# voidstrike/FPSG

Measured on AMD Instinct MI355X. Metric: episodes/sec (+ Chamfer-kernel HBM GB/s in roofline.hbm), 2048-pt clouds, 224x224 images; episode = fwd + Chamfer + bwd, step = E episodes + all-reduce + Adam, higher is better.
Workload: dtype f32

## Files before the change

fpsg_amd/csrc/conv_first.hip:

```cpp
#include "fpsg_common.h"

namespace fpsg {
namespace {

constexpr int kFirstThreads = 256;

struct FoldArgs {
  const float* y;
  const float* chan;
  const float* coef;
  const float* pre_bias;
};

template <int PX, bool FOLD>
__global__ __launch_bounds__(kFirstThreads) void conv_first_dw_kernel(const float* __restrict__ x,
                                                                      const float* __restrict__ dy, FoldArgs fa, int H, int W,
                                                                      int segs_per_row, int n_segs,
                                                                      float* __restrict__ part ) {
  constexpr int LD = PX + 4;
  constexpr int VPR = PX / 4;
  constexpr int NV = 64 * VPR / kFirstThreads;
  constexpr int PE = 9 * (PX + 2);
  constexpr int NP = (PE + kFirstThreads - 1) / kFirstThreads;
  static_assert(64 * VPR % kFirstThreads == 0, "tile vectors divide over the threads");
  __shared__ float dyt[64 * LD];
  __shared__ float xt[9 * LD];
  const int tid = threadIdx.x, lane = tid & 63, wave = tid >> 6;
  const int kk = lane >> 4, col = lane & 15;
  int boff[2];
  bool bval[2];
#pragma unroll
  for (int nt = 0; nt < 2; ++nt) {
    const int tap = 16 * nt + col;
    bval[nt] = tap < 27;
    const int t = bval[nt] ? tap : 0;
    boff[nt] = (t / 3) * LD + (t % 3);
  }
  int vch[NV], vq4[NV], pcr[NP], pj[NP];
#pragma unroll
  for (int it = 0; it < NV; ++it) {
    const int v = it * kFirstThreads + tid;
    vch[it] = v / VPR;
    vq4[it] = (v - vch[it] * VPR) * 4;
  }
#pragma unroll
  for (int it = 0; it < NP; ++it) {
    const int e = it * kFirstThreads + tid;
    pcr[it] = e < PE ? e / (PX + 2) : -1;
    pj[it] = e - (e / (PX + 2)) * (PX + 2);
  }
  v4f rv[NV];
  v4f ry[FOLD ? NV : 1];
  float rp[NP];
  float fsc[FOLD ? NV : 1], fsh[FOLD ? NV : 1], fk1[FOLD ? NV : 1], fk2[FOLD ? NV : 1], fk3[FOLD ? NV : 1], fb[FOLD ? NV : 1];
  if constexpr (FOLD) {
#pragma unroll
    for (int it = 0; it < NV; ++it) {
      const int c = vch[it];
      fsc[it] = fa.chan[c]; fsh[it] = fa.chan[64 + c];
      fk1[it] = fa.coef[c]; fk2[it] = fa.coef[64 + c]; fk3[it] = fa.coef[128 + c];
      fb[it] = fa.pre_bias ? fa.pre_bias[c] : 0.0f;
    }
  }
  auto fetch = [&](int seg) {
    const int row = seg / segs_per_row;
    const int w0 = (seg - row * segs_per_row) * PX;
    const int n = row / H;
    const int h = row - n * H;
#pragma unroll
    for (int it = 0; it < NV; ++it) {
      rv[it] = (v4f){0.0f, 0.0f, 0.0f, 0.0f};
      if constexpr (FOLD) ry[it] = rv[it];
      if (w0 + vq4[it] < W) {
        const size_t o = (((size_t)n * 64 + vch[it]) * H + h) * W + w0 + vq4[it];
        rv[it] = *reinterpret_cast<const v4f*>(dy + o);
        if constexpr (FOLD) ry[it] = *reinterpret_cast<const v4f*>(fa.y + o);
      } else if constexpr (FOLD) {
        ry[it] = (v4f){-3.0e38f, -3.0e38f, -3.0e38f, -3.0e38f};
      }
    }
#pragma unroll
    for (int it = 0; it < NP; ++it) {
      const int c = pcr[it] / 3, r = pcr[it] - 3 * c;
      const int hh = h + r - 1, ww = w0 + pj[it] - 1;
      rp[it] = 0.0f;
      if (pcr[it] >= 0 && hh >= 0 && hh < H && ww >= 0 && ww < W) rp[it] = x[(((size_t)n * 3 + c) * H + hh) * W + ww];
    }
  };
  v4f acc[2] = {{0.0f, 0.0f, 0.0f, 0.0f}, {0.0f, 0.0f, 0.0f, 0.0f}};
  int seg = blockIdx.x;
  if (seg < n_segs) fetch(seg);
  for (; seg < n_segs; seg += gridDim.x) {
    __syncthreads();
#pragma unroll
    for (int it = 0; it < NV; ++it) {
      v4f v = rv[it];
      if constexpr (FOLD) {
#pragma unroll
        for (int u = 0; u < 4; ++u) {
          const float xv = ry[it][u] + fb[it];
          const float dz = rv[it][u] * (fma_rn(xv, fsc[it], fsh[it]) > 0.0f ? 1.0f : 0.0f);
          const float dx = fma_rn(fk1[it], dz, fma_rn(fk2[it], xv, fk3[it]));
          v[u] = ry[it][u] == -3.0e38f ? 0.0f : dx;
        }
      }
      *reinterpret_cast<v4f*>(dyt + vch[it] * LD + vq4[it]) = v;
    }
#pragma unroll
    for (int it = 0; it < NP; ++it)
      if (pcr[it] >= 0) xt[pcr[it] * LD + pj[it]] = rp[it];
    __syncthreads();
    if (seg + (int)gridDim.x < n_segs) fetch(seg + gridDim.x);
    const float* ap = dyt + (16 * wave + col) * LD + kk;
    const float* bp0 = xt + boff[0] + kk;
    const float* bp1 = xt + boff[1] + kk;
#pragma unroll
    for (int s = 0; s < PX / 4; ++s) {
      const float a = ap[4 * s];
      const float b0 = bval[0] ? bp0[4 * s] : 0.0f;
      const float b1 = bval[1] ? bp1[4 * s] : 0.0f;
      acc[0] = __builtin_amdgcn_mfma_f32_16x16x4f32(a, b0, acc[0], 0, 0, 0);
      acc[1] = __builtin_amdgcn_mfma_f32_16x16x4f32(a, b1, acc[1], 0, 0, 0);
    }
  }
  float* pp = part + (size_t)blockIdx.x * 64 * 32;
#pragma unroll
  for (int nt = 0; nt < 2; ++nt)
#pragma unroll
    for (int r = 0; r < 4; ++r) pp[(16 * wave + 4 * kk + r) * 32 + 16 * nt + col] = acc[nt][r];
}

__global__ __launch_bounds__(1024) void conv_first_dw_reduce_kernel(const float* __restrict__ part, int n_part,
                                                                    float* __restrict__ dw ) {
  __shared__ double acc[32][32];
  const int k = blockIdx.x, tap = threadIdx.x & 31, g = threadIdx.x >> 5;
  double a = 0.0;
#pragma unroll 8
  for (int p = g; p < n_part; p += 32) a += (double)part[((size_t)p * 64 + k) * 32 + tap];
  acc[g][tap] = a;
  __syncthreads();
  if (g == 0 && tap < 27) {
    double t = acc[0][tap];
#pragma unroll
    for (int q = 1; q < 32; ++q) t += acc[q][tap];
    dw[k * 27 + tap] = (float)t;
  }
}


__device__ __forceinline__ void first_load_weights(const float* __restrict__ wt, const float* __restrict__ bias, int k,
                                                   float (&w)[27], float& b) {
#pragma unroll
  for (int i = 0; i < 27; ++i) w[i] = wt[k * 27 + i];
  b = bias ? bias[k] : 0.0f;
}

__device__ __forceinline__ void first_wait_weights(const float (&w)[27], float b) {
  asm volatile("" ::"s"(w[0]), "s"(w[15]), "s"(w[23]), "s"(w[25]), "s"(w[26]), "s"(b));
  __builtin_amdgcn_sched_barrier(0);
}

__device__ __forceinline__ void first_channel(const float (&d)[3][3][6], const float (&w)[27], float (&o)[4]) {
#pragma unroll
  for (int p = 0; p < 4; ++p) o[p] = 0.0f;
#pragma unroll
  for (int c = 0; c < 3; ++c)
#pragma unroll
    for (int a = 0; a < 3; ++a)
#pragma unroll
      for (int b = 0; b < 3; ++b) {
        const float wv = w[(c * 3 + a) * 3 + b];
#pragma unroll
        for (int p = 0; p < 4; ++p) o[p] = fma_rn(wv, d[c][a][b + p], o[p]);
      }
}

__device__ __forceinline__ void first_lane_sums(const float (&o)[4], float bk, bool live, float& s0, float& s1) {
  s0 = 0.0f;
  s1 = 0.0f;
#pragma unroll
  for (int p = 0; p < 4; ++p) {
    const float v = o[p] + bk;
    s0 += v;
    s1 = fma_rn(v, v, s1);
  }
  if (!live) s0 = s1 = 0.0f;
}

template <bool STATS, bool NT = false>
__global__ __launch_bounds__(kFirstThreads) void conv_first_fwd_kernel(const float* __restrict__ x,
                                                                       const float* __restrict__ wt , int H,
                                                                       int W, long Q, float* __restrict__ y,
                                                                       const float* __restrict__ bias,
                                                                       float* __restrict__ parts) {
  __shared__ float red[kFirstThreads / 64][64][2];
  const int tid = threadIdx.x, lane = tid & 63, wave = tid >> 6;
  const long q_raw = (long)blockIdx.x * kFirstThreads + tid;
  const bool live = q_raw < Q;
  const long q = live ? q_raw : Q - 1;
  const int W4 = W >> 2;
  const int w4 = (int)(q % W4);
  const long t = q / W4;
  const int h = (int)(t % H);
  const long n = t / H;
  const bool has_left = w4 > 0, has_right = w4 < W4 - 1;
  const bool left_lane = has_left && lane > 0, right_lane = has_right && lane < 63;
  v4f mid[3][3];
  float el[3][3], er[3][3];
  const float* rp[3][3];
  bool rin[3];
#pragma unroll
  for (int a = 0; a < 3; ++a) {
    const int r = h + a - 1;
    rin[a] = r >= 0 && r < H;
    const int rc = rin[a] ? r : h;
#pragma unroll
    for (int c = 0; c < 3; ++c) {
      rp[c][a] = x + (((size_t)n * 3 + c) * H + rc) * W + 4 * w4;
      mid[c][a] = *reinterpret_cast<const v4f*>(rp[c][a]);
      el[c][a] = er[c][a] = 0.0f;
    }
  }
  if (has_left && !left_lane) {
#pragma unroll
    for (int a = 0; a < 3; ++a)
#pragma unroll
      for (int c = 0; c < 3; ++c) el[c][a] = rp[c][a][-1];
  }
  if (has_right && !right_lane) {
#pragma unroll
    for (int a = 0; a < 3; ++a)
#pragma unroll
      for (int c = 0; c < 3; ++c) er[c][a] = rp[c][a][4];
  }
  float d[3][3][6];
#pragma unroll
  for (int c = 0; c < 3; ++c) {
#pragma unroll
    for (int a = 0; a < 3; ++a) {
      v4f m = mid[c][a];
      if (!rin[a]) m = (v4f){0.0f, 0.0f, 0.0f, 0.0f};
      float lft = __shfl_up(m[3], 1, 64), rgt = __shfl_down(m[0], 1, 64);
      if (!left_lane) lft = (has_left && rin[a]) ? el[c][a] : 0.0f;
      if (!right_lane) rgt = (has_right && rin[a]) ? er[c][a] : 0.0f;
      d[c][a][0] = lft; d[c][a][1] = m[0]; d[c][a][2] = m[1]; d[c][a][3] = m[2]; d[c][a][4] = m[3]; d[c][a][5] = rgt;
    }
  }
  const size_t plane = (size_t)H * W;
  float* yp = y + ((size_t)n * 64 * H + h) * W + 4 * w4;
  float wa[27], wb[27], ba = 0.0f, bb = 0.0f;
  first_load_weights(wt, STATS ? bias : nullptr, 0, wa, ba);
  for (int k = 0; k < 64; k += 2) {
    first_wait_weights(wa, ba);
    first_load_weights(wt, STATS ? bias : nullptr, k + 1, wb, bb);
    __builtin_amdgcn_sched_barrier(0);
    float oa[4], ob[4];
    first_channel(d, wa, oa);
    if (live) st_stream<NT>(reinterpret_cast<v4f*>(yp + (size_t)k * plane), (v4f){oa[0], oa[1], oa[2], oa[3]});
    float a0 = 0.0f, a1 = 0.0f, b0 = 0.0f, b1 = 0.0f;
    if (STATS) first_lane_sums(oa, ba, live, a0, a1);
    first_wait_weights(wb, bb);
    first_load_weights(wt, STATS ? bias : nullptr, k + 2 < 64 ? k + 2 : 63, wa, ba);
    __builtin_amdgcn_sched_barrier(0);
    first_channel(d, wb, ob);
    if (live) st_stream<NT>(reinterpret_cast<v4f*>(yp + (size_t)(k + 1) * plane), (v4f){ob[0], ob[1], ob[2], ob[3]});
    if (STATS) {
      first_lane_sums(ob, bb, live, b0, b1);
      wave_sum4_to_last(a0, a1, b0, b1);
      if (lane == 63) {
        *reinterpret_cast<v2f*>(&red[wave][k][0]) = (v2f){a0, a1};
        *reinterpret_cast<v2f*>(&red[wave][k + 1][0]) = (v2f){b0, b1};
      }
    }
  }
  if (STATS) {
    __syncthreads();
    if (tid < 64) {
      float t0 = red[0][tid][0], t1 = red[0][tid][1];
#pragma unroll
      for (int w2 = 1; w2 < kFirstThreads / 64; ++w2) { t0 += red[w2][tid][0]; t1 += red[w2][tid][1]; }
      float* out = parts + ((size_t)tid * gridDim.x + blockIdx.x) * 2;
      out[0] = t0;
      out[1] = t1;
    }
  }
}

}
}

extern "C" size_t fpsg_conv_first_dw_workspace_floats(int N, int H, int W) {
  if (N <= 0 || H <= 0 || W <= 0) return 0;
  return (size_t)2048 * 64 * 32;
}

static int conv_first_dw_launch(const char* fn, const float* x, const float* dy, fpsg::FoldArgs fa, int N, int C, int K,
                                int H, int W, float* dw, float* ws, fpsg_stream_t stream) {
  using namespace fpsg;
  const bool fold = fa.y != nullptr;
  FPSG_REQUIRE(C == 3 && K == 64, FPSG_E_SHAPE, "%s: the 3 -> 64 channel layer only (got %d -> %d)", fn, C, K);
  FPSG_REQUIRE(N > 0 && H > 0 && W > 0 && W % 4 == 0, FPSG_E_SHAPE,
               "%s: N, H positive and W a positive multiple of 4 (got %d,%d,%d)", fn, N, H, W);
  FPSG_REQUIRE_PTR(x); FPSG_REQUIRE_PTR(dy); FPSG_REQUIRE_PTR(dw); FPSG_REQUIRE_PTR(ws);
  FPSG_REQUIRE((reinterpret_cast<uintptr_t>(dy) & 15) == 0 && (reinterpret_cast<uintptr_t>(fa.y) & 15) == 0, FPSG_E_ALIGN,
               "%s: dy / y / ga must be 16-byte aligned", fn);
  hipStream_t s = static_cast<hipStream_t>(stream);
  const int px = W % 112 == 0 ? 112 : 64;
  const int segs_per_row = (W + px - 1) / px;
  const long n_segs_l = (long)N * H * segs_per_row;
  FPSG_REQUIRE(n_segs_l < (1L << 31), FPSG_E_LIMIT, "fpsg_conv_first_dw: %ld row segments beyond the 32-bit walk", n_segs_l);
  const int n_segs = (int)n_segs_l;
  const int resident = px == 112 ? 1024 : 2048;
  const int blocks = n_segs < resident ? n_segs : resident;
  if (px == 112 && fold)
    hipLaunchKernelGGL((conv_first_dw_kernel<112, true>), dim3(blocks), dim3(kFirstThreads), 0, s, x, dy, fa, H, W, segs_per_row, n_segs, ws);
  else if (px == 112)
    hipLaunchKernelGGL((conv_first_dw_kernel<112, false>), dim3(blocks), dim3(kFirstThreads), 0, s, x, dy, fa, H, W, segs_per_row, n_segs, ws);
  else if (fold)
    hipLaunchKernelGGL((conv_first_dw_kernel<64, true>), dim3(blocks), dim3(kFirstThreads), 0, s, x, dy, fa, H, W, segs_per_row, n_segs, ws);
  else
    hipLaunchKernelGGL((conv_first_dw_kernel<64, false>), dim3(blocks), dim3(kFirstThreads), 0, s, x, dy, fa, H, W, segs_per_row, n_segs, ws);
  int rc = launch_status(fn);
  if (rc) return rc;
  hipLaunchKernelGGL(conv_first_dw_reduce_kernel, dim3(64), dim3(1024), 0, s, ws, blocks, dw);
  return launch_status(fn);
}

extern "C" int fpsg_conv_first_dw(const float* x, const float* dy, int N, int C, int K, int H, int W, float* dw,
                                  float* ws, fpsg_stream_t stream) {
  return conv_first_dw_launch("fpsg_conv_first_dw", x, dy, fpsg::FoldArgs{nullptr, nullptr, nullptr, nullptr}, N, C, K, H, W,
                              dw, ws, stream);
}

extern "C" int fpsg_conv_first_dw_fold(const float* x, const float* y, const float* ga, const float* chan,
                                       const float* coef, const float* pre_bias, int N, int C, int K, int H, int W,
                                       float* dw, float* ws, fpsg_stream_t stream) {
  using namespace fpsg;
  FPSG_REQUIRE_PTR(y); FPSG_REQUIRE_PTR(chan); FPSG_REQUIRE_PTR(coef);
  FPSG_REQUIRE(!misaligned4(pre_bias), FPSG_E_ALIGN, "fpsg_conv_first_dw_fold: pre_bias not 4-byte aligned");
  return conv_first_dw_launch("fpsg_conv_first_dw_fold", x, ga, FoldArgs{y, chan, coef, pre_bias}, N, C, K, H, W, dw, ws,
                              stream);
}

extern "C" int fpsg_conv_first_parts(int N, int H, int W) {
  if (N <= 0 || H <= 0 || W <= 0 || W % 4) return 0;
  const long Q = (long)N * H * (W / 4);
  return (int)((Q + fpsg::kFirstThreads - 1) / fpsg::kFirstThreads);
}

extern "C" int fpsg_conv_first_fwd(const float* x, const float* w, int N, int C, int K, int H, int W, float* y,
                                   const float* bias, float* parts, fpsg_stream_t stream) {
  using namespace fpsg;
  FPSG_REQUIRE(C == 3 && K == 64, FPSG_E_SHAPE, "fpsg_conv_first_fwd: the 3 -> 64 channel layer only (got %d -> %d)", C, K);
  FPSG_REQUIRE(N > 0 && H > 0 && W > 0 && W % 4 == 0, FPSG_E_SHAPE,
               "fpsg_conv_first_fwd: N, H positive and W a positive multiple of 4 (got %d,%d,%d)", N, H, W);
  FPSG_REQUIRE_PTR(x); FPSG_REQUIRE_PTR(w); FPSG_REQUIRE_PTR(y);
  FPSG_REQUIRE(((reinterpret_cast<uintptr_t>(x) | reinterpret_cast<uintptr_t>(y)) & 15) == 0, FPSG_E_ALIGN,
               "fpsg_conv_first_fwd: x and y must be 16-byte aligned");
  FPSG_REQUIRE(!misaligned4(bias) && !misaligned4(parts) && !misaligned4(w), FPSG_E_ALIGN,
               "fpsg_conv_first_fwd: w / bias / parts not 4-byte aligned");
  const long Q = (long)N * H * (W / 4);
  const long blocks = (Q + kFirstThreads - 1) / kFirstThreads;
  FPSG_REQUIRE(blocks < (1L << 31), FPSG_E_LIMIT, "fpsg_conv_first_fwd: %ld workgroups beyond the grid limit", blocks);
  hipStream_t s = static_cast<hipStream_t>(stream);
  const bool nt = beyond_cache((size_t)N * 64 * H * W * sizeof(float));
  if (parts && nt)
    hipLaunchKernelGGL((conv_first_fwd_kernel<true, true>), dim3((unsigned)blocks), dim3(kFirstThreads), 0, s, x, w, H, W, Q, y, bias, parts);
  else if (parts)
    hipLaunchKernelGGL(conv_first_fwd_kernel<true>, dim3((unsigned)blocks), dim3(kFirstThreads), 0, s, x, w, H, W, Q, y, bias, parts);
  else if (nt)
    hipLaunchKernelGGL((conv_first_fwd_kernel<false, true>), dim3((unsigned)blocks), dim3(kFirstThreads), 0, s, x, w, H, W, Q, y, nullptr, nullptr);
  else
    hipLaunchKernelGGL(conv_first_fwd_kernel<false>, dim3((unsigned)blocks), dim3(kFirstThreads), 0, s, x, w, H, W, Q, y, nullptr, nullptr);
  return launch_status("fpsg_conv_first_fwd");
}
```

fpsg_amd/csrc/winograd_fused.hip:

```cpp
#include <type_traits>

#include "fpsg_common.h"

namespace fpsg {
namespace {

constexpr int kFusedThreads = 256;
constexpr int kSteps = 16;
constexpr int kUldsFloats = 36 * kSteps * 64;

__device__ __forceinline__ float from_left_or(float keep, float v) {
  return __int_as_float(__builtin_amdgcn_update_dpp(__float_as_int(keep), __float_as_int(v), 0x111, 0xF, 0xF, false));
}
__device__ __forceinline__ float from_right_or(float keep, float v) {
  return __int_as_float(__builtin_amdgcn_update_dpp(__float_as_int(keep), __float_as_int(v), 0x101, 0xF, 0xF, false));
}
__device__ __forceinline__ void in4(const float (&d)[6], float c0, float (&t)[6]) {
  const float p = fma_rn(-4.0f, d[2], d[4]), q = fma_rn(-4.0f, d[1], d[3]);
  const float r = d[4] - d[2], s = d[3] - d[1];
  t[0] = fma_rn(c0, d[0], fma_rn(-5.0f, d[2], d[4]));
  t[1] = p + q;
  t[2] = p - q;
  t[3] = fma_rn(2.0f, s, r);
  t[4] = fma_rn(-2.0f, s, r);
  t[5] = fma_rn(4.0f, d[1], fma_rn(-5.0f, d[3], d[5]));
}
__device__ __forceinline__ void out4(const float (&m)[6], float (&s)[4]) {
  const float p12 = m[1] + m[2], m12 = m[1] - m[2], p34 = m[3] + m[4], m34 = m[3] - m[4];
  s[0] = (m[0] + p12) + p34;
  s[1] = fma_rn(2.0f, m34, m12);
  s[2] = fma_rn(4.0f, p34, p12);
  s[3] = fma_rn(8.0f, m34, m12) + m[5];
}

template <bool ACT, bool STATS, bool NT = false>
__global__ __launch_bounds__(kFusedThreads) void wino4_fused_c64_kernel(const float* __restrict__ x,
                                                                        const float* __restrict__ U ,
                                                                        int K, int H, int W, int Th, int Tw, long P,
                                                                        int S, float* __restrict__ y,
                                                                        const float* __restrict__ chan,
                                                                        const float* __restrict__ pre_bias,
                                                                        const float* __restrict__ out_bias,
                                                                        float* __restrict__ parts) {
  extern __shared__ __attribute__((aligned(16))) float ulds[];
  constexpr int C = 64;
  float* actp = ulds + kUldsFloats;
  const int tid = threadIdx.x, lane = tid & 63, wave = tid >> 6;
  const int kk = lane >> 4, col = lane & 15;
  const int i = blockIdx.x;
  const int slice = (i >> 3) % S;
  const int j = (i & 7) + 8 * (i / (8 * S));
  const int per_slice = gridDim.x / S;
  const int k0 = slice * 16;
  {
    const int kl = tid >> 4, c4 = tid & 15;
    const float* up = U + ((size_t)k0 + kl) * C + 4 * c4;
    v4f ub[36];
#pragma unroll
    for (int xi = 0; xi < 36; ++xi) ub[xi] = *reinterpret_cast<const v4f*>(up + (size_t)xi * K * C);
#pragma unroll
    for (int kq = 0; kq < 4; ++kq) {
      v4f* dst = reinterpret_cast<v4f*>(ulds + ((size_t)c4 * 64 + kq * 16 + kl) * 36);
#pragma unroll
      for (int x4 = 0; x4 < 9; ++x4)
        dst[x4] = (v4f){ub[4 * x4][kq], ub[4 * x4 + 1][kq], ub[4 * x4 + 2][kq], ub[4 * x4 + 3][kq]};
    }
  }
  if (ACT && tid < C) {
    actp[tid] = chan[tid];
    actp[C + tid] = chan[C + tid];
    actp[2 * C + tid] = pre_bias ? pre_bias[tid] : 0.0f;
  }
  __syncthreads();
  const __amdgpu_buffer_rsrc_t xrsrc = __builtin_amdgcn_make_buffer_rsrc(
      const_cast<float*>(x), 0, (int)(P * 16 * C * sizeof(float)), 0x00020000);
  float st0[4] = {0.0f, 0.0f, 0.0f, 0.0f}, st1[4] = {0.0f, 0.0f, 0.0f, 0.0f}, ob[4] = {0.0f, 0.0f, 0.0f, 0.0f};
  if (STATS && out_bias) {
#pragma unroll
    for (int r = 0; r < 4; ++r) ob[r] = out_bias[k0 + 4 * kk + r];
  }
  const long G = (P + 15) >> 4;
  struct Tile {
    uint32_t boff[6], eoffb[6];
    float c4t, mb, c4l, mr, mr5;
    int tw, th;
    unsigned n;
    bool live;
  };
  auto locate = [&](long g, Tile& t) {
    const long p_raw = g * 16 + col;
    t.live = p_raw < P;
    const long p = t.live ? p_raw : P - 1;
    const unsigned pu = (unsigned)p;
    t.tw = (int)(pu % (unsigned)Tw);
    const unsigned q = pu / (unsigned)Tw;
    t.th = (int)(q % (unsigned)Th);
    t.n = q / (unsigned)Th;
    const bool has_left = t.tw > 0, has_right = t.tw < Tw - 1;
    const bool edge_l = has_left && col == 0, edge_r = has_right && col == 15;
    const int r0 = 4 * t.th - 1;
    const bool top_in = r0 >= 0, bot_in = r0 + 5 < H;
    t.c4t = top_in ? 4.0f : 0.0f;
    t.mb = bot_in ? 1.0f : 0.0f;
    t.c4l = has_left ? 4.0f : 0.0f;
    t.mr = has_right ? 1.0f : 0.0f;
    t.mr5 = t.mr * t.mb;
    const uint32_t lane_elem = (uint32_t)((((size_t)t.n * C + kk) * H) * W + 4 * t.tw);
    const uint32_t eadd = edge_l ? (uint32_t)-4 : (edge_r ? 16u : 0u);
#pragma unroll
    for (int r = 0; r < 6; ++r) {
      const int row = r0 + r;
      t.boff[r] = (lane_elem + (uint32_t)((row < 0 ? 0 : (row >= H ? H - 1 : row)) * W)) * 4u;
      t.eoffb[r] = t.boff[r] + eadd;
    }
  };
  const uint32_t step_bytes = (uint32_t)(4 * H * W) * 4u;
  struct Raw { v4f mid[6]; float e[6]; };
  auto load_raw = [&](const Tile& t, int c4, Raw& w) {
    const uint32_t sbase = (uint32_t)c4 * step_bytes;
#pragma unroll
    for (int r = 0; r < 6; ++r) {
      w.mid[r] = __builtin_bit_cast(v4f, __builtin_amdgcn_raw_buffer_load_b128(xrsrc, t.boff[r], sbase, 0));
      w.e[r] = __uint_as_float(__builtin_amdgcn_raw_buffer_load_b32(xrsrc, t.eoffb[r], sbase, 0));
    }
  };
  const long g_stride = 4L * per_slice;
  Tile cur, nxt;
  Raw ra, rb;
  long g = (long)j * 4 + wave;
  if (g < G) {
    locate(g, cur);
    load_raw(cur, 0, ra);
    load_raw(cur, 1, rb);
  }
  for (; g < G; g += g_stride) {
    locate(g + g_stride < G ? g + g_stride : g, nxt);
    const float c4t = cur.c4t, mb = cur.mb, c4l = cur.c4l, mr = cur.mr, mr5 = cur.mr5;
    const bool live = cur.live;
    const int tw = cur.tw, th = cur.th;
    const unsigned n = cur.n;
    v4f acc[36];

    auto compute = [&](int c4, const Raw& w, v4f (&accr)[36], auto first) {
      v4f a[9];
      {
        const v4f* up = reinterpret_cast<const v4f*>(ulds + ((size_t)c4 * 64 + lane) * 36);
#pragma unroll
        for (int q4 = 0; q4 < 9; ++q4) a[q4] = up[q4];
      }
      __builtin_amdgcn_sched_barrier(0);
      float asc = 1.0f, ash = 0.0f, apb = 0.0f;
      if (ACT) { asc = actp[4 * c4 + kk]; ash = actp[C + 4 * c4 + kk]; apb = actp[2 * C + 4 * c4 + kk]; }
      float d[6][6];
#pragma unroll
      for (int r = 0; r < 6; ++r) {
        float m0 = w.mid[r][0], m1 = w.mid[r][1], m2 = w.mid[r][2], m3 = w.mid[r][3], e = w.e[r];
        if (ACT) {
          m0 = __builtin_fmaxf(fma_rn(m0 + apb, asc, ash), 0.0f);
          m1 = __builtin_fmaxf(fma_rn(m1 + apb, asc, ash), 0.0f);
          m2 = __builtin_fmaxf(fma_rn(m2 + apb, asc, ash), 0.0f);
          m3 = __builtin_fmaxf(fma_rn(m3 + apb, asc, ash), 0.0f);
          e = __builtin_fmaxf(fma_rn(e + apb, asc, ash), 0.0f);
        }
        const float lft = from_left_or(e, m3);
        d[r][0] = r == 5 ? lft * mb : lft;
        d[r][5] = from_right_or(e, m0) * (r == 5 ? mr5 : mr);
        d[r][1] = r == 5 ? m0 * mb : m0;
        d[r][2] = r == 5 ? m1 * mb : m1;
        d[r][3] = r == 5 ? m2 * mb : m2;
        d[r][4] = r == 5 ? m3 * mb : m3;
      }
      float t[6][6];
#pragma unroll
      for (int j = 0; j < 6; ++j) {
        const float colv[6] = {d[0][j], d[1][j], d[2][j], d[3][j], d[4][j], d[5][j]};
        in4(colv, c4t, t[j]);
      }
#pragma unroll
      for (int i = 0; i < 6; ++i) {
        const float rowv[6] = {t[0][i], t[1][i], t[2][i], t[3][i], t[4][i], t[5][i]};
        float o[6];
        in4(rowv, c4l, o);
        {
          const int x0 = 6 * i, l0 = x0;
#define FPSG_A(c) a[(l0 + (c)) >> 2][(l0 + (c)) & 3]
          if constexpr (decltype(first)::value) {
            asm volatile(
                "s_nop 1\n\t"
                "v_mfma_f32_16x16x4_f32 %0, %6, %12, 0\n\t"
                "v_mfma_f32_16x16x4_f32 %1, %7, %13, 0\n\t"
                "v_mfma_f32_16x16x4_f32 %2, %8, %14, 0\n\t"
                "v_mfma_f32_16x16x4_f32 %3, %9, %15, 0\n\t"
                "v_mfma_f32_16x16x4_f32 %4, %10, %16, 0\n\t"
                "v_mfma_f32_16x16x4_f32 %5, %11, %17, 0"
                : "=&a"(accr[x0]), "=&a"(accr[x0 + 1]), "=&a"(accr[x0 + 2]), "=&a"(accr[x0 + 3]), "=&a"(accr[x0 + 4]),
                  "=&a"(accr[x0 + 5])
                : "v"(FPSG_A(0)), "v"(FPSG_A(1)), "v"(FPSG_A(2)), "v"(FPSG_A(3)), "v"(FPSG_A(4)), "v"(FPSG_A(5)),
                  "v"(o[0]), "v"(o[1]), "v"(o[2]), "v"(o[3]), "v"(o[4]), "v"(o[5]));
          } else {
            asm volatile(
                "s_nop 1\n\t"
                "v_mfma_f32_16x16x4_f32 %0, %6, %12, %0\n\t"
                "v_mfma_f32_16x16x4_f32 %1, %7, %13, %1\n\t"
                "v_mfma_f32_16x16x4_f32 %2, %8, %14, %2\n\t"
                "v_mfma_f32_16x16x4_f32 %3, %9, %15, %3\n\t"
                "v_mfma_f32_16x16x4_f32 %4, %10, %16, %4\n\t"
                "v_mfma_f32_16x16x4_f32 %5, %11, %17, %5"
                : "+a"(accr[x0]), "+a"(accr[x0 + 1]), "+a"(accr[x0 + 2]), "+a"(accr[x0 + 3]), "+a"(accr[x0 + 4]),
                  "+a"(accr[x0 + 5])
                : "v"(FPSG_A(0)), "v"(FPSG_A(1)), "v"(FPSG_A(2)), "v"(FPSG_A(3)), "v"(FPSG_A(4)), "v"(FPSG_A(5)),
                  "v"(o[0]), "v"(o[1]), "v"(o[2]), "v"(o[3]), "v"(o[4]), "v"(o[5]));
          }
#undef FPSG_A
        }
      }
    };
#define FPSG_LOAD(st, buf) load_raw(cur, st, buf); __builtin_amdgcn_sched_barrier(0)
#define FPSG_LOAD_NEXT(st, buf) load_raw(nxt, st, buf); __builtin_amdgcn_sched_barrier(0)
#define FPSG_COMPUTE(st, buf) compute(st, buf, acc, std::false_type{}); __builtin_amdgcn_sched_barrier(0)
#define FPSG_COMPUTE_FIRST(st, buf) compute(st, buf, acc, std::true_type{}); __builtin_amdgcn_sched_barrier(0)
    __builtin_amdgcn_sched_barrier(0);
    FPSG_COMPUTE_FIRST(0, ra);
    FPSG_LOAD(2, ra);
    FPSG_COMPUTE(1, rb);
    FPSG_LOAD(3, rb);
#pragma unroll 1
    for (int c4 = 2; c4 < kSteps - 2; c4 += 2) {
      FPSG_COMPUTE(c4, ra);
      FPSG_LOAD(c4 + 2, ra);
      FPSG_COMPUTE(c4 + 1, rb);
      FPSG_LOAD(c4 + 3, rb);
    }
    FPSG_COMPUTE(kSteps - 2, ra);
    FPSG_LOAD_NEXT(0, ra);
    FPSG_COMPUTE(kSteps - 1, rb);
    FPSG_LOAD_NEXT(1, rb);
#undef FPSG_COMPUTE
#undef FPSG_COMPUTE_FIRST
#undef FPSG_LOAD_NEXT
#undef FPSG_LOAD
    asm volatile("s_nop 15\n\ts_nop 15" ::: "memory");
    __builtin_amdgcn_sched_barrier(0);
#pragma unroll
    for (int r = 0; r < 4; ++r) {
      float s[6][4];
#pragma unroll
      for (int c = 0; c < 6; ++c) {
        float m[6];
#pragma unroll
        for (int a = 0; a < 6; ++a) m[a] = acc[6 * a + c][r];
        out4(m, s[c]);
      }
      if (live) {
        float* yp = y + ((((size_t)n * K + k0 + 4 * kk + r) * H) + 4 * th) * W + 4 * tw;
#pragma unroll
        for (int a = 0; a < 4; ++a) {
          float rowv[6], o[4];
#pragma unroll
          for (int c = 0; c < 6; ++c) rowv[c] = s[c][a];
          out4(rowv, o);
          st_stream<NT>(reinterpret_cast<v4f*>(yp + (size_t)a * W), (v4f){o[0], o[1], o[2], o[3]});
          if (STATS) {
#pragma unroll
            for (int u = 0; u < 4; ++u) {
              const float v = o[u] + ob[r];
              st0[r] += v;
              st1[r] = fma_rn(v, v, st1[r]);
            }
          }
        }
      }
    }
    cur = nxt;
  }
  if (STATS) {
    __syncthreads();
#pragma unroll
    for (int r = 0; r < 4; ++r) {
      float a0 = st0[r], a1 = st1[r];
      a0 += __uint_as_float(lane_xor<1>(__float_as_uint(a0))); a1 += __uint_as_float(lane_xor<1>(__float_as_uint(a1)));
      a0 += __uint_as_float(lane_xor<2>(__float_as_uint(a0))); a1 += __uint_as_float(lane_xor<2>(__float_as_uint(a1)));
      a0 += __uint_as_float(lane_xor<4>(__float_as_uint(a0))); a1 += __uint_as_float(lane_xor<4>(__float_as_uint(a1)));
      a0 += __uint_as_float(lane_xor<8>(__float_as_uint(a0))); a1 += __uint_as_float(lane_xor<8>(__float_as_uint(a1)));
      if (col == 0) {
        ulds[((wave * 4 + kk) * 4 + r) * 2] = a0;
        ulds[((wave * 4 + kk) * 4 + r) * 2 + 1] = a1;
      }
    }
    __syncthreads();
    if (tid < 16) {
      float t0 = 0.0f, t1 = 0.0f;
#pragma unroll
      for (int w = 0; w < 4; ++w) { t0 += ulds[(w * 16 + tid) * 2]; t1 += ulds[(w * 16 + tid) * 2 + 1]; }
      float* out = parts + ((size_t)(k0 + tid) * per_slice + j) * 2;
      out[0] = t0;
      out[1] = t1;
    }
  }
}

}
}

static long wino_fused_per_slice(long P, int S) {
  const long G = (P + 15) / 16;
  long per_slice = (256 + S - 1) / S;
  const long need = (G + 3) / 4;
  if (per_slice > need) per_slice = need;
  return ((per_slice + 7) / 8) * 8;
}

static int wino_conv_fused_launch(const char* fn, const float* x, const float* chan, const float* pre_bias,
                                  const float* U, int N, int C, int K, int H, int W, float* y, const float* out_bias,
                                  float* parts, fpsg_stream_t stream) {
  using namespace fpsg;
  FPSG_REQUIRE(C == 64, FPSG_E_SHAPE, "%s: C must be 64 (got %d)", fn, C);
  FPSG_REQUIRE(N > 0 && K > 0 && K % 16 == 0 && K <= 1024 && H > 0 && W > 0 && H % 4 == 0 && W % 4 == 0, FPSG_E_SHAPE,
               "%s: K a positive multiple of 16 (<= 1024), H and W positive multiples of 4 "
               "(got K=%d H=%d W=%d)", fn, K, H, W);
  FPSG_REQUIRE_PTR(x); FPSG_REQUIRE_PTR(U); FPSG_REQUIRE_PTR(y);
  FPSG_REQUIRE(((reinterpret_cast<uintptr_t>(x) | reinterpret_cast<uintptr_t>(y) | reinterpret_cast<uintptr_t>(U)) & 15) == 0,
               FPSG_E_ALIGN, "%s: x, y and U must be 16-byte aligned", fn);
  FPSG_REQUIRE(!misaligned4(out_bias) && !misaligned4(parts), FPSG_E_ALIGN, "%s: out_bias / parts not 4-byte aligned", fn);
  FPSG_REQUIRE((size_t)N * C * H * W * sizeof(float) < ((size_t)1 << 32), FPSG_E_LIMIT,
               "%s: x must be below 4 GiB (32-bit lane offsets; got N=%d H=%d W=%d)", fn, N, H, W);
  const long P = (long)N * (H / 4) * (W / 4);
  const int S = K / 16;
  const size_t lds_bytes = (size_t)(kUldsFloats + 3 * 64) * sizeof(float);
  typedef void (*kern_t)(const float*, const float*, int, int, int, int, int, long, int, float*, const float*,
                         const float*, const float*, float*);
  const bool nt = beyond_cache((size_t)N * K * H * W * sizeof(float));
  const kern_t kern =
      nt ? (chan ? (parts ? wino4_fused_c64_kernel<true, true, true> : wino4_fused_c64_kernel<true, false, true>)
                 : (parts ? wino4_fused_c64_kernel<false, true, true> : wino4_fused_c64_kernel<false, false, true>))
         : (chan ? (parts ? wino4_fused_c64_kernel<true, true> : wino4_fused_c64_kernel<true, false>)
                 : (parts ? wino4_fused_c64_kernel<false, true> : wino4_fused_c64_kernel<false, false>));
  const hipError_t lds_optin = hipFuncSetAttribute(reinterpret_cast<const void*>(kern),
                                                   hipFuncAttributeMaxDynamicSharedMemorySize, 160 * 1024);
  if (lds_optin != hipSuccess) {
    set_error("%s: cannot reserve %zu B of LDS: %s", fn, lds_bytes, hipGetErrorString(lds_optin));
    return static_cast<int>(lds_optin);
  }
  dim3 grid((unsigned)(wino_fused_per_slice(P, S) * S));
  hipLaunchKernelGGL(kern, grid, dim3(kFusedThreads), lds_bytes, static_cast<hipStream_t>(stream), x, U, K, H, W, H / 4,
                     W / 4, P, S, y, chan, pre_bias, out_bias, parts);
  return launch_status(fn);
}

extern "C" int fpsg_wino_conv_fused(const float* x, const float* U, int N, int C, int K, int H, int W, float* y,
                                    fpsg_stream_t stream) {
  return wino_conv_fused_launch("fpsg_wino_conv_fused", x, nullptr, nullptr, U, N, C, K, H, W, y, nullptr, nullptr, stream);
}

extern "C" int fpsg_wino_conv_fused_act(const float* x, const float* chan, const float* pre_bias, const float* U,
                                        int N, int C, int K, int H, int W, float* y, fpsg_stream_t stream) {
  using namespace fpsg;
  FPSG_REQUIRE_PTR(chan);
  FPSG_REQUIRE(!misaligned4(pre_bias), FPSG_E_ALIGN, "fpsg_wino_conv_fused_act: pre_bias not 4-byte aligned");
  return wino_conv_fused_launch("fpsg_wino_conv_fused_act", x, chan, pre_bias, U, N, C, K, H, W, y, nullptr, nullptr, stream);
}

extern "C" int fpsg_wino_conv_fused_parts(int N, int K, int H, int W) {
  if (N <= 0 || K <= 0 || K % 16 || H <= 0 || W <= 0 || H % 4 || W % 4) return 0;
  return (int)wino_fused_per_slice((long)N * (H / 4) * (W / 4), K / 16);
}

extern "C" int fpsg_wino_conv_fused_stats(const float* x, const float* chan, const float* pre_bias, const float* U,
                                          int N, int C, int K, int H, int W, float* y, const float* out_bias,
                                          float* parts, fpsg_stream_t stream) {
  using namespace fpsg;
  FPSG_REQUIRE_PTR(parts);
  FPSG_REQUIRE(!misaligned4(pre_bias), FPSG_E_ALIGN, "fpsg_wino_conv_fused_stats: pre_bias not 4-byte aligned");
  return wino_conv_fused_launch("fpsg_wino_conv_fused_stats", x, chan, pre_bias, U, N, C, K, H, W, y, out_bias, parts, stream);
}
```

Measured before the change: 45.39.

## Trim register pressure and address math in first-layer conv weight-gradient kernel

Moves the per-channel fold coefficients from registers into a shared table and raises the occupancy hint for the 112-pixel fold variant. Switches the dy/y/x loads to buffer loads with 32-bit offsets, so out-of-range reads come back as zero and 64-bit address arithmetic is avoided. Handles a small tail of patch elements separately and adds a zero row in shared memory so the MFMA loop no longer needs per-tap predicates. Also turns the Winograd loop into a do-while to drop the entry check. The cost is extra shared-memory reads per tile and a new size limit on H*W.

Result: no change. 45.88, median of 3 (+1.1%).

```diff
diff --git a/fpsg_amd/csrc/conv_first.hip b/fpsg_amd/csrc/conv_first.hip
--- a/fpsg_amd/csrc/conv_first.hip
+++ b/fpsg_amd/csrc/conv_first.hip
@@ -13,35 +13,37 @@
 };
 
 template <int PX, bool FOLD>
-__global__ __launch_bounds__(kFirstThreads) void conv_first_dw_kernel(const float* __restrict__ x,
-                                                                      const float* __restrict__ dy, FoldArgs fa, int H, int W,
-                                                                      int segs_per_row, int n_segs,
-                                                                      float* __restrict__ part ) {
+__global__ __launch_bounds__(kFirstThreads) __attribute__((amdgpu_waves_per_eu(PX == 112 && FOLD ? 4 : 1)))
+void conv_first_dw_kernel(const float* __restrict__ x, const float* __restrict__ dy, FoldArgs fa, int H, int W,
+                          int segs_per_row, int n_segs, float* __restrict__ part ) {
   constexpr int LD = PX + 4;
   constexpr int VPR = PX / 4;
   constexpr int NV = 64 * VPR / kFirstThreads;
   constexpr int PE = 9 * (PX + 2);
-  constexpr int NP = (PE + kFirstThreads - 1) / kFirstThreads;
+  constexpr int REM = PE % kFirstThreads;
+  constexpr bool SREM = REM > 0 && REM <= 4;
+  constexpr int NP = SREM ? PE / kFirstThreads : (PE + kFirstThreads - 1) / kFirstThreads;
   static_assert(64 * VPR % kFirstThreads == 0, "tile vectors divide over the threads");
   __shared__ float dyt[64 * LD];
-  __shared__ float xt[9 * LD];
+  __shared__ float xt[10 * LD];
   const int tid = threadIdx.x, lane = tid & 63, wave = tid >> 6;
   const int kk = lane >> 4, col = lane & 15;
   int boff[2];
-  bool bval[2];
 #pragma unroll
   for (int nt = 0; nt < 2; ++nt) {
     const int tap = 16 * nt + col;
-    bval[nt] = tap < 27;
-    const int t = bval[nt] ? tap : 0;
-    boff[nt] = (t / 3) * LD + (t % 3);
-  }
-  int vch[NV], vq4[NV], pcr[NP], pj[NP];
+    boff[nt] = tap < 27 ? (tap / 3) * LD + (tap % 3) : 9 * LD;
+  }
+  if (tid < LD) xt[9 * LD + tid] = 0.0f;
+  int vch[NV], vq4[NV], vlds[NV], pcr[NP], pj[NP];
+  uint32_t voff[NV];
 #pragma unroll
   for (int it = 0; it < NV; ++it) {
     const int v = it * kFirstThreads + tid;
     vch[it] = v / VPR;
     vq4[it] = (v - vch[it] * VPR) * 4;
+    vlds[it] = vch[it] * LD + vq4[it];
+    voff[it] = ((uint32_t)vch[it] * (uint32_t)(H * W) + (uint32_t)vq4[it]) * 4u;
   }
 #pragma unroll
   for (int it = 0; it < NP; ++it) {
@@ -52,14 +54,13 @@
   v4f rv[NV];
   v4f ry[FOLD ? NV : 1];
   float rp[NP];
-  float fsc[FOLD ? NV : 1], fsh[FOLD ? NV : 1], fk1[FOLD ? NV : 1], fk2[FOLD ? NV : 1], fk3[FOLD ? NV : 1], fb[FOLD ? NV : 1];
+  float rs[SREM ? REM : 1];
+  __shared__ float ctab[FOLD ? 6 * 64 : 1];
   if constexpr (FOLD) {
-#pragma unroll
-    for (int it = 0; it < NV; ++it) {
-      const int c = vch[it];
-      fsc[it] = fa.chan[c]; fsh[it] = fa.chan[64 + c];
-      fk1[it] = fa.coef[c]; fk2[it] = fa.coef[64 + c]; fk3[it] = fa.coef[128 + c];
-      fb[it] = fa.pre_bias ? fa.pre_bias[c] : 0.0f;
+    if (tid < 64) {
+      ctab[tid] = fa.chan[tid]; ctab[64 + tid] = fa.chan[64 + tid];
+      ctab[128 + tid] = fa.coef[tid]; ctab[192 + tid] = fa.coef[64 + tid]; ctab[256 + tid] = fa.coef[128 + tid];
+      ctab[320 + tid] = fa.pre_bias ? fa.pre_bias[tid] : 0.0f;
     }
   }
   auto fetch = [&](int seg) {
@@ -67,14 +68,19 @@
     const int w0 = (seg - row * segs_per_row) * PX;
     const int n = row / H;
     const int h = row - n * H;
+    const size_t seg0 = (((size_t)n * 64) * H + h) * W + w0;
+    const int tile_bytes = (int)((64u * (uint32_t)(H * W) - (uint32_t)(h * W + w0)) * 4u);
+    const __amdgpu_buffer_rsrc_t drsrc = __builtin_amdgcn_make_buffer_rsrc(const_cast<float*>(dy + seg0), 0, tile_bytes, 0x00020000);
+    const __amdgpu_buffer_rsrc_t yrsrc = __builtin_amdgcn_make_buffer_rsrc(const_cast<float*>(FOLD ? fa.y + seg0 : dy + seg0), 0, tile_bytes, 0x00020000);
+    const __amdgpu_buffer_rsrc_t xrsrc = __builtin_amdgcn_make_buffer_rsrc(
+        const_cast<float*>(x + (size_t)n * 3 * H * W), 0, (int)(3u * (uint32_t)(H * W) * 4u), 0x00020000);
 #pragma unroll
     for (int it = 0; it < NV; ++it) {
       rv[it] = (v4f){0.0f, 0.0f, 0.0f, 0.0f};
       if constexpr (FOLD) ry[it] = rv[it];
-      if (w0 + vq4[it] < W) {
-        const size_t o = (((size_t)n * 64 + vch[it]) * H + h) * W + w0 + vq4[it];
-        rv[it] = *reinterpret_cast<const v4f*>(dy + o);
-        if constexpr (FOLD) ry[it] = *reinterpret_cast<const v4f*>(fa.y + o);
+      if (PX == 112 || w0 + vq4[it] < W) {
+        rv[it] = __builtin_bit_cast(v4f, __builtin_amdgcn_raw_buffer_load_b128(drsrc, voff[it], 0, 0));
+        if constexpr (FOLD) ry[it] = __builtin_bit_cast(v4f, __builtin_amdgcn_raw_buffer_load_b128(yrsrc, voff[it], 0, 0));
       } else if constexpr (FOLD) {
         ry[it] = (v4f){-3.0e38f, -3.0e38f, -3.0e38f, -3.0e38f};
       }
@@ -83,8 +89,21 @@
     for (int it = 0; it < NP; ++it) {
       const int c = pcr[it] / 3, r = pcr[it] - 3 * c;
       const int hh = h + r - 1, ww = w0 + pj[it] - 1;
-      rp[it] = 0.0f;
-      if (pcr[it] >= 0 && hh >= 0 && hh < H && ww >= 0 && ww < W) rp[it] = x[(((size_t)n * 3 + c) * H + hh) * W + ww];
+      const bool in = (pcr[it] >= 0) & ((unsigned)hh < (unsigned)H) & ((unsigned)ww < (unsigned)W);
+      const uint32_t xo = in ? (uint32_t)((c * H + hh) * W + ww) * 4u : 0u;
+      const float xv = __uint_as_float(__builtin_amdgcn_raw_buffer_load_b32(xrsrc, xo, 0, 0));
+      rp[it] = in ? xv : 0.0f;
+    }
+    if constexpr (SREM) {
+#pragma unroll
+      for (int k = 0; k < REM; ++k) {
+        constexpr int cr0 = (NP * kFirstThreads) / (PX + 2), j0 = (NP * kFirstThreads) % (PX + 2);
+        const int cr = cr0 + (j0 + k) / (PX + 2), j = (j0 + k) % (PX + 2);
+        const int c = cr / 3, r = cr - 3 * c;
+        const int hh = h + r - 1, ww = w0 + j - 1;
+        rs[k] = 0.0f;
+        if (hh >= 0 && hh < H && ww >= 0 && ww < W) rs[k] = x[(((size_t)n * 3 + c) * H + hh) * W + ww];
+      }
     }
   };
   v4f acc[2] = {{0.0f, 0.0f, 0.0f, 0.0f}, {0.0f, 0.0f, 0.0f, 0.0f}};
@@ -96,19 +115,28 @@
     for (int it = 0; it < NV; ++it) {
       v4f v = rv[it];
       if constexpr (FOLD) {
+        const float* ct = ctab + vch[it];
+        const float fsc = ct[0], fsh = ct[64], fk1 = ct[128], fk2 = ct[192], fk3 = ct[256], fb = ct[320];
 #pragma unroll
         for (int u = 0; u < 4; ++u) {
-          const float xv = ry[it][u] + fb[it];
-          const float dz = rv[it][u] * (fma_rn(xv, fsc[it], fsh[it]) > 0.0f ? 1.0f : 0.0f);
-          const float dx = fma_rn(fk1[it], dz, fma_rn(fk2[it], xv, fk3[it]));
-          v[u] = ry[it][u] == -3.0e38f ? 0.0f : dx;
+          const float xv = ry[it][u] + fb;
+          const float dz = rv[it][u] * (fma_rn(xv, fsc, fsh) > 0.0f ? 1.0f : 0.0f);
+          const float dx = fma_rn(fk1, dz, fma_rn(fk2, xv, fk3));
+          v[u] = PX != 112 && ry[it][u] == -3.0e38f ? 0.0f : dx;
         }
       }
-      *reinterpret_cast<v4f*>(dyt + vch[it] * LD + vq4[it]) = v;
+      *reinterpret_cast<v4f*>(dyt + vlds[it]) = v;
     }
 #pragma unroll
     for (int it = 0; it < NP; ++it)
       if (pcr[it] >= 0) xt[pcr[it] * LD + pj[it]] = rp[it];
+    if constexpr (SREM) {
+#pragma unroll
+      for (int k = 0; k < REM; ++k) {
+        constexpr int cr0 = (NP * kFirstThreads) / (PX + 2), j0 = (NP * kFirstThreads) % (PX + 2);
+        if (tid == k) xt[(cr0 + (j0 + k) / (PX + 2)) * LD + (j0 + k) % (PX + 2)] = rs[k];
+      }
+    }
     __syncthreads();
     if (seg + (int)gridDim.x < n_segs) fetch(seg + gridDim.x);
     const float* ap = dyt + (16 * wave + col) * LD + kk;
@@ -117,8 +145,8 @@
 #pragma unroll
     for (int s = 0; s < PX / 4; ++s) {
       const float a = ap[4 * s];
-      const float b0 = bval[0] ? bp0[4 * s] : 0.0f;
-      const float b1 = bval[1] ? bp1[4 * s] : 0.0f;
+      const float b0 = bp0[4 * s];
+      const float b1 = bp1[4 * s];
       acc[0] = __builtin_amdgcn_mfma_f32_16x16x4f32(a, b0, acc[0], 0, 0, 0);
       acc[1] = __builtin_amdgcn_mfma_f32_16x16x4f32(a, b1, acc[1], 0, 0, 0);
     }
@@ -302,6 +330,8 @@
   FPSG_REQUIRE(N > 0 && H > 0 && W > 0 && W % 4 == 0, FPSG_E_SHAPE,
                "%s: N, H positive and W a positive multiple of 4 (got %d,%d,%d)", fn, N, H, W);
   FPSG_REQUIRE_PTR(x); FPSG_REQUIRE_PTR(dy); FPSG_REQUIRE_PTR(dw); FPSG_REQUIRE_PTR(ws);
+  FPSG_REQUIRE((size_t)H * W < ((size_t)1 << 24), FPSG_E_LIMIT,
+               "%s: one image's dy must be below 4 GiB (32-bit lane offsets; got H=%d W=%d)", fn, H, W);
   FPSG_REQUIRE((reinterpret_cast<uintptr_t>(dy) & 15) == 0 && (reinterpret_cast<uintptr_t>(fa.y) & 15) == 0, FPSG_E_ALIGN,
                "%s: dy / y / ga must be 16-byte aligned", fn);
   hipStream_t s = static_cast<hipStream_t>(stream);
diff --git a/fpsg_amd/csrc/winograd_fused.hip b/fpsg_amd/csrc/winograd_fused.hip
--- a/fpsg_amd/csrc/winograd_fused.hip
+++ b/fpsg_amd/csrc/winograd_fused.hip
@@ -224,13 +224,15 @@
     FPSG_LOAD(2, ra);
     FPSG_COMPUTE(1, rb);
     FPSG_LOAD(3, rb);
+    int c4 = 2;
 #pragma unroll 1
-    for (int c4 = 2; c4 < kSteps - 2; c4 += 2) {
+    do {
       FPSG_COMPUTE(c4, ra);
       FPSG_LOAD(c4 + 2, ra);
       FPSG_COMPUTE(c4 + 1, rb);
       FPSG_LOAD(c4 + 3, rb);
-    }
+      c4 += 2;
+    } while (c4 < kSteps - 2);
     FPSG_COMPUTE(kSteps - 2, ra);
     FPSG_LOAD_NEXT(0, ra);
     FPSG_COMPUTE(kSteps - 1, rb);
```
